# Sanasar1/Learning-Deep-Neural-Network-In-Distributed-Computing-Environment

Measured on AMD Instinct MI355X. Metric: samples/sec (whole node) + DP scaling eff., 3-layer MLP at 1/2/4/8 MI355X, higher is better.
Workload: dtype bf16

## Files before the change

learning-deep-neural-network-in-distributed-computing-environment_amd/csrc/bindings.cpp:

```cpp
#include <torch/extension.h>
#include <pybind11/stl.h>
#include <vector>
#include <cstring>
#include <string>
#include <mutex>
#include <map>
#include <ATen/hip/impl/HIPGuardImplMasqueradingAsCUDA.h>
#include <ATen/hip/impl/HIPStreamMasqueradingAsCUDA.h>

#include <rocprofiler-sdk-roctx/roctx.h>
#include "ldnn_kernels.h"

namespace {

hipStream_t cur_stream(const at::Tensor& t) {
  return c10::hip::getCurrentHIPStreamMasqueradingAsCUDA(t.device().index()).stream();
}

void check(hipError_t e, const char* what) {
  TORCH_CHECK(e == hipSuccess, "ldnn kernel '", what, "' failed: ", hipGetErrorString(e));
}

void check_dev(const at::Tensor& t, at::ScalarType dt, const char* name) {
  TORCH_CHECK(t.is_cuda(), name, " must be a GPU tensor");
// ... 950 lines not shown
  p.dlogits = bf16_mut(dlogits);
  p.stats = stats.data_ptr<float>();
  p.B = (int)B;
  p.C = (int)num_classes;
  p.ld = 16;
  p.grad_scale = (float)grad_scale;
  c10::hip::HIPGuardMasqueradingAsCUDA g(parts.device());
  check(ldnn::head_xent_parts(p, parts.data_ptr<float>(), (int)parts.size(0), cur_stream(parts)), "head_xent_parts");
}

void head_dgrad_stream(const at::Tensor& h, const at::Tensor& W, const at::Tensor& dlogits, const at::Tensor& dh,
                       const c10::optional<at::Tensor>& dbias, int64_t dgrad_epi) {
  check_dev(h, at::kBFloat16, "h");
  check_dev(W, at::kBFloat16, "W");
  check_dev(dlogits, at::kBFloat16, "dlogits");
  check_dev(dh, at::kBFloat16, "dh");
  const int64_t B = h.size(0), K = h.size(1);
  TORCH_CHECK(h.dim() == 2 && h.stride(1) == 1 && h.stride(0) % 8 == 0 && K % 8 == 0 && aligned16(h.data_ptr()),
              "head_dgrad_stream: h must be [B][K] with 16-B aligned rows");
  TORCH_CHECK(W.dim() == 2 && W.size(0) <= 16 && W.size(1) == K && W.stride(1) == 1 && W.stride(0) % 8 == 0 &&
                  aligned16(W.data_ptr()),
              "head_dgrad_stream: W must be [<= 16][K] with 16-B aligned rows");
  TORCH_CHECK(dlogits.is_contiguous() && dlogits.dim() == 2 && dlogits.size(0) == B && dlogits.size(1) == 16,
              "head_dgrad_stream: dlogits must be a contiguous [B][16] buffer");
  TORCH_CHECK(dh.dim() == 2 && dh.size(0) == B && dh.size(1) == K && dh.stride(1) == 1 && dh.stride(0) % 8 == 0 &&
                  aligned16(dh.data_ptr()),
              "head_dgrad_stream: dh must be [B][K] with 16-B aligned rows");
  TORCH_CHECK(dgrad_epi == ldnn::EPI_NONE || dgrad_epi == ldnn::EPI_DRELU || dgrad_epi == ldnn::EPI_DSIGMOID,
              "head_dgrad_stream: dgrad_epi must be EPI_NONE / EPI_DRELU / EPI_DSIGMOID");
  ldnn::HeadParams p{};
  p.h = bf16_ptr(h);
  p.W = bf16_ptr(W);
  p.dlogits = bf16_mut(dlogits);
  p.B = (int)B;
  p.K = (int)K;
  p.ld = 16;
  p.ldh = (int)h.stride(0);
  p.ldw = (int)W.stride(0);
  p.ldw_rows = (int)W.size(0);
  p.dh = bf16_mut(dh);
  p.lddh = (int)dh.stride(0);
  p.dgrad_epi = (int)dgrad_epi;
  if (dbias.has_value()) {
    check_dev(*dbias, at::kFloat, "dbias");
    TORCH_CHECK(dbias->is_contiguous() && dbias->numel() >= K, "head_dgrad_stream: bad dbias");
    p.dbias = dbias->data_ptr<float>();
  }
  c10::hip::HIPGuardMasqueradingAsCUDA g(h.device());
  check(ldnn::head_dgrad_stream(p, cur_stream(h)), "head_dgrad_stream");
}

void head_bwd(const at::Tensor& h, const at::Tensor& W, const at::Tensor& dlogits, const at::Tensor& dh,
              const at::Tensor& dW, const c10::optional<at::Tensor>& dbias, int64_t dgrad_epi,
              const c10::optional<at::Tensor>& db) {
  check_dev(h, at::kBFloat16, "h");
  check_dev(W, at::kBFloat16, "W");
  check_dev(dlogits, at::kBFloat16, "dlogits");
  check_dev(dh, at::kBFloat16, "dh");
  check_dev(dW, at::kFloat, "dW");
  const int64_t B = h.size(0), K = h.size(1);
  TORCH_CHECK(h.dim() == 2 && h.stride(1) == 1 && h.stride(0) % 8 == 0 && K % 64 == 0 && aligned16(h.data_ptr()),
              "head_bwd: h must be [B][K] with K % 64 == 0 and 16-B aligned rows");
  TORCH_CHECK(W.dim() == 2 && W.size(0) <= 16 && W.size(1) == K && W.stride(1) == 1, "head_bwd: W must be [<= 16][K]");
  TORCH_CHECK(dlogits.is_contiguous() && dlogits.dim() == 2 && dlogits.size(0) == B && dlogits.size(1) == 16 &&
                  aligned16(dlogits.data_ptr()),
              "head_bwd: dlogits must be a contiguous [B][16] buffer");
  TORCH_CHECK(dh.dim() == 2 && dh.size(0) == B && dh.size(1) == K && dh.stride(1) == 1 && dh.stride(0) % 8 == 0 &&
                  aligned16(dh.data_ptr()),
              "head_bwd: dh must be [B][K] with 16-B aligned rows");
  TORCH_CHECK(dgrad_epi == ldnn::EPI_NONE || dgrad_epi == ldnn::EPI_DRELU, "head_bwd: dgrad_epi must be EPI_NONE / EPI_DRELU");
  TORCH_CHECK(dW.dim() == 2 && dW.size(1) == K && dW.size(0) <= 16 && dW.stride(1) == 1, "head_bwd: dW must be [<= 16][K]");
  ldnn::HeadParams p{};
  p.h = bf16_ptr(h);
  p.W = bf16_ptr(W);
  p.dlogits = bf16_mut(dlogits);
  p.B = (int)B;
  p.K = (int)K;
  p.ld = 16;
  p.ldh = (int)h.stride(0);
  p.ldw = (int)W.stride(0);
  p.ldw_rows = (int)W.size(0);
  p.dh = bf16_mut(dh);
  p.lddh = (int)dh.stride(0);
  p.dgrad_epi = (int)dgrad_epi;
  p.dW = dW.data_ptr<float>();
  p.lddw = (int)dW.stride(0);
  p.nrows_w = (int)dW.size(0);
  if (dbias.has_value()) {
    check_dev(*dbias, at::kFloat, "dbias");
    TORCH_CHECK(dbias->is_contiguous() && dbias->numel() >= K, "head_bwd: bad dbias");
    p.dbias = dbias->data_ptr<float>();
  }
  if (db.has_value()) {
    check_dev(*db, at::kFloat, "db");
    TORCH_CHECK(db->is_contiguous() && db->numel() >= dW.size(0), "head_bwd: bad db");
    p.db = db->data_ptr<float>();
  }
  c10::hip::HIPGuardMasqueradingAsCUDA g(h.device());
  check(ldnn::head_bwd(p, cur_stream(h)), "head_bwd");
}

void head_wgrad(const at::Tensor& dz, const at::Tensor& h, const at::Tensor& dW, const c10::optional<at::Tensor>& db,
                int64_t splits) {
  check_dev(dz, at::kBFloat16, "dz");
  check_dev(h, at::kBFloat16, "h");
  check_dev(dW, at::kFloat, "dW");
  const int64_t B = h.size(0), K = h.size(1), ld = dz.size(1);
  TORCH_CHECK(dz.is_contiguous() && dz.size(0) == B && ld % 16 == 0 && ld <= 64, "head_wgrad: dz [B][ld], ld % 16 == 0");
  TORCH_CHECK(h.stride(1) == 1 && h.stride(0) % 8 == 0 && K % 8 == 0 && aligned16(h.data_ptr()), "head_wgrad: bad h");
  TORCH_CHECK(dW.dim() == 2 && dW.size(1) == K && dW.stride(1) == 1 && dW.size(0) <= ld && dW.stride(0) % 4 == 0 &&
                  aligned16(dW.data_ptr()),
              "head_wgrad: dW must be [rows <= ld][K] with 16-B aligned rows");
  ldnn::HeadWgradParams p{};
  p.dz = bf16_ptr(dz);
  p.h = bf16_ptr(h);
  p.dW = dW.data_ptr<float>();
  if (db.has_value()) {
    check_dev(*db, at::kFloat, "db");
    TORCH_CHECK(db->is_contiguous() && db->numel() >= dW.size(0), "head_wgrad: bad db");
    p.db = db->data_ptr<float>();
  }
  p.B = (int)B;
  p.K = (int)K;
  p.ld = (int)ld;
  p.ldh = (int)h.stride(0);
  p.lddw = (int)dW.stride(0);
  p.nrows = (int)dW.size(0);
  c10::hip::HIPGuardMasqueradingAsCUDA g(h.device());
  check(ldnn::head_wgrad(p, (int)splits, cur_stream(h)), "head_wgrad");
}

void bump_step(const at::Tensor& hp, const c10::optional<at::Tensor>& clip) {
  check_dev(hp, at::kFloat, "hp");
  TORCH_CHECK(hp.is_contiguous() && hp.numel() >= 2, "bump_step: hp must hold [lr, step]");
  check(ldnn::bump_step(hp.data_ptr<float>(), cur_stream(hp), clip_ptr(clip, hp)), "bump_step");
}

float* ema_hdr(const char* fn, const at::Tensor& hdr, const at::Tensor* like) {
  check_dev(hdr, at::kFloat, "hdr");
  TORCH_CHECK(hdr.is_contiguous() && hdr.numel() >= ldnn::kEmaState &&
                  (like == nullptr || hdr.device() == like->device()),
              fn, ": hdr must be a contiguous fp32 header of ", (int)ldnn::kEmaState,
              " elements on the buffers' device");
  return hdr.data_ptr<float>();
}

void ema_begin(const at::Tensor& hdr, const c10::optional<at::Tensor>& clip) {
  float* h = ema_hdr("ema_begin", hdr, nullptr);
  check(ldnn::ema_begin(h, cur_stream(hdr), clip_ptr(clip, hdr)), "ema_begin");
}

void lr_sched(const at::Tensor& hdr, const at::Tensor& hp, const c10::optional<at::Tensor>& clip) {
// ... 1207 lines not shown
        py::arg("chunks"), py::arg("partials"), py::arg("hp"), py::arg("grad_scale"), py::arg("beta1"),
        py::arg("beta2"), py::arg("eps"), py::arg("weight_decay"), py::arg("ranges"), py::arg("seg_offsets"),
        py::arg("clip") = py::none(), py::arg("policy") = (int64_t)1);
  m.def("lamb_finalize", &lamb_finalize, "per-segment LAMB trust ratios |w| / |u| and norms from lamb_moments' partials "
        "(+ ext sums); sums_out: the [2S] sums alone", py::arg("partials"), py::arg("segtab"), py::arg("ratio"),
        py::arg("w_norm"), py::arg("u_norm"), py::arg("ext") = py::none(), py::arg("clip") = py::none(),
        py::arg("sums_out") = py::none());
  m.def("lamb_apply", &lamb_apply, "LAMB apply pass: w -= lr * ratio * u over a 64-aligned range (+ bf16 shadow, "
        "gradient zero ranges)", py::arg("param"), py::arg("grad"), py::arg("m"), py::arg("v"), py::arg("shadow"),
        py::arg("hp"), py::arg("beta1"), py::arg("beta2"), py::arg("eps"), py::arg("weight_decay"), py::arg("ratio"),
        py::arg("map"), py::arg("zero_ranges") = std::vector<std::pair<int64_t, int64_t>>{},
        py::arg("clip") = py::none());
  m.def("adam_step", &adam_step, py::arg("param"), py::arg("grad"), py::arg("m"), py::arg("v"),
        py::arg("shadow"), py::arg("hp"), py::arg("grad_scale"), py::arg("beta1"), py::arg("beta2"),
        py::arg("eps"), py::arg("weight_decay"), py::arg("decoupled"),
        py::arg("zero_ranges") = std::vector<std::pair<int64_t, int64_t>>{}, py::arg("clip") = py::none());
  m.def("lion_step", &lion_step, "Lion: w = w (1 - lr wd) - lr sign(beta1 m + (1 - beta1) g), m = beta2 m + "
        "(1 - beta2) g (+ bf16 shadow, gradient zero ranges); lr = hp[0]", py::arg("param"), py::arg("grad"),
        py::arg("exp_avg"), py::arg("shadow"), py::arg("hp"), py::arg("grad_scale"), py::arg("beta1"),
        py::arg("beta2"), py::arg("weight_decay"),
        py::arg("zero_ranges") = std::vector<std::pair<int64_t, int64_t>>{}, py::arg("clip") = py::none());
  m.def("bump_step", &bump_step, py::arg("hp"), py::arg("clip") = py::none());
  m.def("lr_sched", &lr_sched, "learning-rate schedule, once per step: hp[0] = base * s(t + 1), the factor and the "
        "step count into hdr (nothing on a skipped step)", py::arg("hdr"), py::arg("hp"), py::arg("clip") = py::none());
  m.def("ema_begin", &ema_begin, "weight EMA, once per step: a_t and the update count into hdr (not on a skipped step)",
        py::arg("hdr"), py::arg("clip") = py::none());
  m.def("ema_update", &ema_update, "ema += a_t * (master - ema), a_t read from hdr", py::arg("master"),
        py::arg("ema"), py::arg("hdr"));
  m.def("ema_swap", &ema_swap, "master <-> ema (exact), shadow = bf16(new master)", py::arg("master"), py::arg("ema"),
        py::arg("shadow") = py::none());
  m.def("grad_sumsq", &grad_sumsq, "per-workgroup sums of squares of a flat fp32 range into partials[slot0 ...]; "
        "returns the number of slots written", py::arg("grad"), py::arg("partials"), py::arg("slot0") = 0);
  m.def("grad_sumsq_parts", &ldnn::grad_sumsq_parts, py::arg("n"));
  m.def("sumsq_total", &sumsq_total, py::arg("partials"), py::arg("nparts"), py::arg("out"));
  m.def("clip_finalize", &clip_finalize, "global-norm clipping state (coef / skip / norm / counters) from the "
        "partials (+ an external sum of squares)", py::arg("partials"), py::arg("nparts"), py::arg("state"),
        py::arg("grad_scale"), py::arg("ext") = py::none());
  m.def("set_opt_max_blocks", &ldnn::set_opt_max_blocks, py::arg("n"),
        "grid cap of optimizer launches from now on (0 = default)");
  m.def("head_fwd_xent", &head_fwd_xent, "fused narrow Linear + softmax-xent + argmax (per-16-row stats slots)",
        py::arg("h"), py::arg("W"), py::arg("bias"), py::arg("labels"), py::arg("logits"), py::arg("dlogits"),
        py::arg("stats"), py::arg("num_classes"), py::arg("grad_scale"), py::arg("dh") = py::none(), py::arg("dbias") = py::none(),
        py::arg("dgrad_epi") = (int64_t)ldnn::EPI_DRELU, py::arg("dbias_ws") = py::none(),
        py::arg("dgrad_mode") = (int64_t)-1);
  m.def("head_dgrad_ws_floats", &ldnn::head_dgrad_ws_floats, py::arg("B"), py::arg("K"));
  m.def("head_xent_parts", &head_xent_parts, "softmax-xent + argmax from EPI_BIAS_RELU_HEAD partial logits",
        py::arg("parts"), py::arg("bias"), py::arg("labels"), py::arg("logits"), py::arg("dlogits"), py::arg("stats"),
        py::arg("num_classes"), py::arg("grad_scale"));
  m.def("head_dgrad_stream", &head_dgrad_stream, "streaming head dgrad: dh = (dlogits W) * act'(h), dbias += colsums",
        py::arg("h"), py::arg("W"), py::arg("dlogits"), py::arg("dh"), py::arg("dbias") = py::none(),
        py::arg("dgrad_epi") = (int64_t)ldnn::EPI_DRELU);
  m.def("head_bwd", &head_bwd, "fused head dgrad + wgrad (dW / db / dbias accumulated: pre-cleared)", py::arg("h"),
        py::arg("W"), py::arg("dlogits"), py::arg("dh"), py::arg("dW"), py::arg("dbias") = py::none(),
        py::arg("dgrad_epi") = (int64_t)ldnn::EPI_DRELU, py::arg("db") = py::none());
  m.def("head_wgrad", &head_wgrad, "dW = dz^T h (+ db = colsum dz); splits > 1 accumulate atomically",
        py::arg("dz"), py::arg("h"), py::arg("dW"), py::arg("db") = py::none(), py::arg("splits") = 0);
  m.def("head_dgrad_max_k", &ldnn::head_dgrad_max_k);
  m.def("head_wgrad_splits", &ldnn::head_wgrad_splits, py::arg("B"), py::arg("K"));
  m.def("bn_fwd", &bn_fwd, py::arg("x"), py::arg("y"), py::arg("residual"), py::arg("gamma"), py::arg("beta"),
        py::arg("running_mean"), py::arg("running_var"), py::arg("save_mean"), py::arg("save_invstd"),
        py::arg("ws"), py::arg("eps"), py::arg("momentum"), py::arg("training"), py::arg("relu"),
        py::arg("num_batches") = py::none(), py::arg("stats_ready") = false, py::arg("mask") = py::none());
  m.def("bn_workspace_floats", &ldnn::bn_workspace_floats, "fp32 workspace of one BatchNorm (zero it once, keep it)",
        py::arg("C"));
  m.def("bn_bwd", &bn_bwd, py::arg("x"), py::arg("y"), py::arg("dy"), py::arg("dx"), py::arg("dres"),
        py::arg("gamma"), py::arg("save_mean"), py::arg("save_invstd"), py::arg("ws"), py::arg("dgamma"),
        py::arg("dbeta"), py::arg("relu"), py::arg("mask") = py::none(), py::arg("grad_assign") = false,
        py::arg("dy2") = py::none(), py::arg("stats_ready") = false);
  m.def("pool_fwd", &pool_fwd, py::arg("x"), py::arg("y"), py::arg("argmax"), py::arg("R"), py::arg("S"),
        py::arg("stride"), py::arg("pad"), py::arg("is_max"), py::arg("nchw_out") = false);
  m.def("pool_bwd", &pool_bwd, py::arg("dy"), py::arg("argmax"), py::arg("dx"), py::arg("R"), py::arg("S"),
        py::arg("stride"), py::arg("pad"), py::arg("is_max"), py::arg("dy2") = py::none(),
        py::arg("nchw_dy") = false);
  m.def("bn_dual_fwd", &bn_dual_fwd, "y = relu(bn_a(x) + bn_b(r)) in one pass (the shortcut BN output never stored)",
        py::arg("x"), py::arg("r"), py::arg("y"), py::arg("mask"), py::arg("gamma_a"), py::arg("beta_a"),
        py::arg("rm_a"), py::arg("rv_a"), py::arg("mean_a"), py::arg("invstd_a"), py::arg("ws_a"), py::arg("eps_a"),
        py::arg("mom_a"), py::arg("nb_a"), py::arg("ready_a"), py::arg("gamma_b"), py::arg("beta_b"),
        py::arg("rm_b"), py::arg("rv_b"), py::arg("mean_b"), py::arg("invstd_b"), py::arg("ws_b"), py::arg("eps_b"),
        py::arg("mom_b"), py::arg("nb_b"), py::arg("ready_b"));
  m.def("bn_dual_bwd", &bn_dual_bwd, "backward of bn_dual_fwd: dx, dr and both BNs' dgamma / dbeta",
        py::arg("x"), py::arg("r"), py::arg("y"), py::arg("mask"), py::arg("dy"), py::arg("dy2"), py::arg("dx"),
        py::arg("dr"), py::arg("gamma_a"), py::arg("mean_a"), py::arg("invstd_a"), py::arg("ws_a"),
        py::arg("dgamma_a"), py::arg("dbeta_a"), py::arg("assign_a"), py::arg("gamma_b"), py::arg("mean_b"),
        py::arg("invstd_b"), py::arg("ws_b"), py::arg("dgamma_b"), py::arg("dbeta_b"), py::arg("assign_b"));
  m.def("bn_pool_fwd", &bn_pool_fwd, "relu(BN(x)) -> 3x3/2 max-pool in one pass (pooled output + argmax)",
        py::arg("x"), py::arg("y"), py::arg("argmax"), py::arg("gamma"), py::arg("beta"), py::arg("running_mean"),
        py::arg("running_var"), py::arg("save_mean"), py::arg("save_invstd"), py::arg("ws"), py::arg("eps"),
        py::arg("momentum"), py::arg("num_batches") = py::none(), py::arg("stats_ready") = false,
        py::arg("pad") = 1, py::arg("xam") = py::none());
  m.def("bn_pool_bwd", &bn_pool_bwd, "backward of bn_pool_fwd: dx, dgamma / dbeta", py::arg("x"), py::arg("dy"),
        py::arg("argmax"), py::arg("dx"), py::arg("gamma"), py::arg("save_mean"), py::arg("save_invstd"),
        py::arg("ws"), py::arg("dgamma"), py::arg("dbeta"), py::arg("grad_assign") = false,
        py::arg("dy2") = py::none(), py::arg("pad") = 1, py::arg("xam") = py::none());
  m.def("gap_fwd", &gap_fwd);
  m.def("gap_bwd", &gap_bwd);
  m.def("set_conv_combine_last", &ldnn::set_conv_combine_last,
        "split-K combine summer: 1 = the tile's last K slice, 0 = the last workgroup to arrive", py::arg("on"));
  m.def("get_conv_combine_last", &ldnn::get_conv_combine_last);
  m.def("set_conv_bn_bwd", &ldnn::set_conv_bn_bwd,
        "dgrad-side BN backward statistics: 0 off, 1 slab sum only (default), 2 also the dgrad epilogue");
  m.def("get_conv_bn_bwd", &ldnn::get_conv_bn_bwd);
  m.def("gap_linear_ok", &ldnn::gap_linear_ok, "shapes the fused pooled classifier head takes", py::arg("N"),
        py::arg("HW"), py::arg("C"), py::arg("ncls"));
  m.def("gap_linear_fwd", &gap_linear_fwd, "global average pool + Linear (<= 16 classes) in one launch", py::arg("x"),
        py::arg("w"), py::arg("b"), py::arg("pooled"), py::arg("logits"), py::arg("ncls"));
  m.def("gap_linear_bwd", &gap_linear_bwd, "its backward: dW, db and the input gradient in one launch", py::arg("g"),
        py::arg("pooled"), py::arg("w"), py::arg("dw"), py::arg("db"), py::arg("dx"), py::arg("ncls"),
// ... 50 lines not shown
```

learning-deep-neural-network-in-distributed-computing-environment_amd/csrc/include/ldnn_kernels.h:

```cpp
#pragma once
#include <hip/hip_runtime.h>
#include <stdint.h>

namespace ldnn {

enum Epilogue : int {
  EPI_NONE = 0,
  EPI_BIAS = 1,
  EPI_BIAS_RELU = 2,
  EPI_BIAS_SIGMOID = 3,
  EPI_DRELU = 4,
  EPI_DSIGMOID = 5,
  EPI_OPT_SGD = 6,
  EPI_OPT_ADAM = 7,
  EPI_BIAS_RELU_MASK = 8,
  EPI_DRELU_MASK = 9,
  EPI_BIAS_RELU_HEAD = 10,
};

struct OptEpi {
  float* master;
  float* m;
  float* v;
  uint16_t* shadow;
// ... 302 lines not shown
int grad_sumsq_parts(int64_t n);
hipError_t grad_sumsq(const float* grad, int64_t n, float* partials, hipStream_t s);
hipError_t sumsq_total(const float* partials, int nparts, float* out, hipStream_t s);
hipError_t clip_finalize(const float* partials, int nparts, const float* ext, float* state, float grad_scale,
                         hipStream_t s);

int seg_sumsq_chunk();
hipError_t seg_sumsq(const float* master, const float* grad, int64_t n, const int32_t* chunks, int nchunks,
                     float* partials, hipStream_t s);
hipError_t trust_finalize(bool lamb, const float* partials, int nchunks, const int32_t* segtab, int S,
                          const float* ext, const float* hdr, const float* clip, float grad_scale, float weight_decay,
                          float* ratio, float* w_norm, float* g_norm, float* sums_out, hipStream_t s);

struct LambParams {
  float beta1, beta2, eps, weight_decay;
  GradZero zero;
};
hipError_t lamb_moments(const float* master, const float* grad, float* m, float* v, int64_t n, const int32_t* chunks,
                        int nchunks, const float* hp, float grad_scale, LambParams lp, float* partials,
                        hipStream_t s, const float* clip = nullptr, int policy = 1);
hipError_t lamb_apply(float* param, float* grad, const float* m, const float* v, uint16_t* shadow, const float* hp,
                      LambParams lp, int64_t n, const float* ratio, const uint16_t* map, hipStream_t s,
                      const float* clip = nullptr);

hipError_t lr_sched(float* hdr, float* hp, hipStream_t s, const float* clip = nullptr);

hipError_t ema_begin(float* hdr, hipStream_t s, const float* clip = nullptr);
hipError_t ema_update(const float* master, float* ema, const float* hdr, int64_t n, hipStream_t s);
hipError_t ema_swap(float* master, float* ema, uint16_t* shadow, int64_t n, hipStream_t s);

struct HeadParams {
  const uint16_t* h;
  const uint16_t* W;
  const float* bias;
  const int64_t* labels;
  uint16_t* logits;
  uint16_t* dlogits;
  float* stats;
  int B, K, C, ld, ldh, ldw, ldw_rows;
  float grad_scale;
  uint16_t* dh;
  float* dbias;
  float* dbias_ws;
  int lddh, dgrad_epi;
  int dgrad_mode;
  float* dW;
  float* db;
  int lddw, nrows_w;
};
hipError_t head_fwd_xent(const HeadParams& p, hipStream_t s);
hipError_t head_xent_parts(const HeadParams& p, const float* parts, int nparts, hipStream_t s);
hipError_t head_dgrad_stream(const HeadParams& p, hipStream_t s);
hipError_t head_bwd(const HeadParams& p, hipStream_t s);
int head_dgrad_max_k();
size_t head_dgrad_ws_floats(int B, int K);
hipError_t slab_sum(const float* ws, float* out, int64_t n4, int splits, float beta, hipStream_t s);
struct HeadWgradParams {
  const uint16_t* dz;
  const uint16_t* h;
  float* dW;
  float* db;
  int B, K, ld, ldh, lddw, nrows;
};
hipError_t head_wgrad(const HeadWgradParams& p, int splits, hipStream_t s);
int head_wgrad_splits(int B, int K);

hipError_t synth_normal_bf16(uint16_t* x, int64_t n, uint64_t seed, float stddev, hipStream_t s);
hipError_t synth_labels(int64_t* y, int64_t n, int classes, uint64_t seed, hipStream_t s);

constexpr int kAugOps = 15, kAugBins = 10, kAugPolicySlots = 64;
struct AugParams {
  const uint8_t* images;
  const int64_t* index;
  void* out;
  const float* a;
  const float* b;
  int64_t n_images;
  int B, C, H, W;
  uint64_t seed;
  int mode;
  int pad;
  int fixed_op, fixed_bin, fixed_sign;
  int n_policies;
  float mags[kAugOps][kAugBins];
  float rot_cos[kAugBins], rot_sin[kAugBins];
  int pol_op[kAugPolicySlots];
  float pol_prob[kAugPolicySlots];
  int pol_bin[kAugPolicySlots];
  int signed_op[kAugOps];
};
constexpr int kAugMaxPixels = 28 * 1024;
hipError_t augment_batch(const AugParams& p, bool out_f32, hipStream_t s);


constexpr int kIpcMaxRanks = 8;
constexpr int kIpcMaxBlocks = 256;
struct IpcPeers {
  const char* data[kIpcMaxRanks];
  uint32_t* sig[kIpcMaxRanks];
  char* mine;
  uint32_t* ctr;
  int* err;
  size_t half_bytes;
};
hipError_t oneshot_all_reduce(const IpcPeers& p, int rank, int world, int64_t n, bool bf16, void* buf, int blocks,
                              hipStream_t s);
// ... 3 lines not shown
```

learning-deep-neural-network-in-distributed-computing-environment_amd/csrc/kernels/head.hip:

```cpp
#include <algorithm>

#include <cstdlib>

#include "ldnn_common.h"
#include "ldnn_gemm_tile.h"
#include "ldnn_kernels.h"

namespace ldnn {

namespace {

constexpr int kFwdWaves = 8;

constexpr int kHeadDgradMaxK = 4096;

__device__ __forceinline__ int hs_off(int r, int q, int K) {
  return r * ((K + 127) & ~127) * 2 + ((q ^ (r & 15)) << 4);
}

template <int NT, bool DG>
__device__ __forceinline__ void head_softmax_xent(const HeadParams& p, floatx4 (&acc)[NT], floatx4 (*red)[NT][64],
                                                  int nred, float* dls, int lane, int row, int slot) {
#pragma unroll
  for (int j = 0; j < NT; ++j)
// ... 424 lines not shown
}

template <int DEPI>
hipError_t head_dgrad_dispatch(const HeadParams& p, hipStream_t s) {
  if (p.dgrad_mode == 0) {
    hipError_t e = launch_head_fwd<-1, false>(p, s);
    if (e != hipSuccess) return e;
    return launch_head_dgrad_stream<DEPI>(p, s);
  }
  hipError_t e = launch_head_fwd_dg<DEPI>(p, s);
  if (e != hipSuccess || p.dbias == nullptr) return e;
  return slab_sum(p.dbias_ws, p.dbias, p.K / 4, (p.B + 15) / 16, 1.f, s);
}

}

hipError_t head_fwd_xent(const HeadParams& p, hipStream_t s) {
  if (p.B <= 0) return hipSuccess;
  if (p.ld > 64 || p.ld % 16 != 0 || p.C > p.ld || p.ldw_rows > p.ld || p.K % 8 != 0) return hipErrorInvalidValue;
  if (p.dh == nullptr) return launch_head_fwd<-1, false>(p, s);
  if (p.lddh % 8 != 0) return hipErrorInvalidValue;
  if (p.dgrad_mode < 0 || p.dgrad_mode > 2 || (p.dgrad_mode == 0 && p.ld != 16)) return hipErrorInvalidValue;
  if ((p.dgrad_mode == 1 || p.dgrad_mode == 2) &&
      (p.K > kHeadDgradMaxK || (p.dbias != nullptr && p.dbias_ws == nullptr)))
    return hipErrorInvalidValue;
  switch (p.dgrad_epi) {
    case EPI_NONE: return head_dgrad_dispatch<EPI_NONE>(p, s);
    case EPI_DRELU: return head_dgrad_dispatch<EPI_DRELU>(p, s);
    case EPI_DSIGMOID: return head_dgrad_dispatch<EPI_DSIGMOID>(p, s);
    default: return hipErrorInvalidValue;
  }
}

hipError_t head_xent_parts(const HeadParams& p, const float* parts, int nparts, hipStream_t s) {
  if (p.B <= 0) return hipSuccess;
  if (p.ld != 16 || p.C > 16 || nparts < 1 || parts == nullptr) return hipErrorInvalidValue;
  const int slots = (p.B + 15) / 16;
  head_xent_parts_kernel<<<(slots + kPartWaves - 1) / kPartWaves, kPartWaves * 64, 0, s>>>(p, parts, nparts);
  return hipGetLastError();
}

hipError_t head_dgrad_stream(const HeadParams& p, hipStream_t s) {
  if (p.B <= 0) return hipSuccess;
  if (p.ld != 16 || p.dh == nullptr || p.lddh % 8 != 0 || p.K % 8 != 0 || p.ldw_rows > 16) return hipErrorInvalidValue;
  switch (p.dgrad_epi) {
    case EPI_NONE: return launch_head_dgrad_stream<EPI_NONE>(p, s);
    case EPI_DRELU: return launch_head_dgrad_stream<EPI_DRELU>(p, s);
    case EPI_DSIGMOID: return launch_head_dgrad_stream<EPI_DSIGMOID>(p, s);
    default: return hipErrorInvalidValue;
  }
}

typedef short s16x4 __attribute__((ext_vector_type(4)));
constexpr int kHbUnroll = 4;

template <bool RELU>
__global__ __launch_bounds__(256) void head_bwd_kernel(HeadParams p, int rows_per_wg) {
  constexpr int kH = 16 * 128, kD = 16 * 32, kSt = kH + kD;
  constexpr int kWave = kHbUnroll * kSt;
  __shared__ __attribute__((aligned(16))) char smem[4 * kWave];
  static_assert(4 * kWave >= 4 * 64 * 17 * 4, "the reduction scratch fits");
  const int lane = threadIdx.x & 63, wid = threadIdx.x >> 6;
  const int g = lane >> 4, r16 = lane & 15;
  const int n0 = blockIdx.x * 64;
  const int r_begin = blockIdx.y * rows_per_wg, r_end = min(p.B, r_begin + rows_per_wg);
  char* const st = smem + wid * kWave;
  typedef __attribute__((address_space(3))) bf16x4 lds_b4;

  s16x4 wa[4];
#pragma unroll
  for (int t = 0; t < 4; ++t) {
    const int n = n0 + (t >> 1) * 32 + 8 * (r16 >> 2) + (t & 1) * 4 + (r16 & 3);
#pragma unroll
    for (int q = 0; q < 4; ++q) {
      const int c = 4 * g + q;
      wa[t][q] = (c < p.ldw_rows && n < p.K) ? (short)p.W[(size_t)c * p.ldw + n] : (short)0;
    }
  }
  floatx4 acc2[4];
#pragma unroll
  for (int t = 0; t < 4; ++t) acc2[t] = floatx4{0.f, 0.f, 0.f, 0.f};
  float cs[16];
#pragma unroll
  for (int k = 0; k < 16; ++k) cs[k] = 0.f;
  float dbs[4] = {0.f, 0.f, 0.f, 0.f};
  const int q = r16 >> 2, pp = r16 & 3;

  for (int mb = r_begin + wid * 16; mb < r_end; mb += 64 * kHbUnroll) {
    u16x8 hv[kHbUnroll][2];
    uint2 dl[kHbUnroll];
#pragma unroll
    for (int u = 0; u < kHbUnroll; ++u) {
      const int m = mb + u * 64 + r16;
      hv[u][0] = hv[u][1] = u16x8{0, 0, 0, 0, 0, 0, 0, 0};
      dl[u] = uint2{0u, 0u};
      if (m < r_end) {
        const bf16_t* hr = p.h + (size_t)m * p.ldh + n0 + 8 * g;
        hv[u][0] = *reinterpret_cast<const u16x8*>(hr);
        hv[u][1] = *reinterpret_cast<const u16x8*>(hr + 32);
        dl[u] = *reinterpret_cast<const uint2*>(p.dlogits + (size_t)m * 16 + 4 * g);
      }
    }
#pragma unroll
    for (int u = 0; u < kHbUnroll; ++u) {
      char* sb = st + u * kSt;
      *reinterpret_cast<u16x8*>(sb + r16 * 128 + ((g ^ (r16 & 7)) << 4)) = hv[u][0];
      *reinterpret_cast<u16x8*>(sb + r16 * 128 + (((4 + g) ^ (r16 & 7)) << 4)) = hv[u][1];
      *reinterpret_cast<uint2*>(sb + kH + r16 * 32 + ((g ^ ((r16 >> 2) & 3)) << 3)) = dl[u];
    }
#pragma unroll
    for (int u = 0; u < kHbUnroll; ++u) {
      const int m = mb + u * 64 + r16;
      const s16x4 bl = __builtin_bit_cast(s16x4, dl[u]);
      floatx4 d[4];
#pragma unroll
      for (int t = 0; t < 4; ++t)
        d[t] = __builtin_amdgcn_mfma_f32_16x16x16bf16_1k(wa[t], bl, floatx4{0.f, 0.f, 0.f, 0.f}, 0, 0, 0);
      u16x8 o[2];
#pragma unroll
      for (int k = 0; k < 16; ++k) {
        const uint16_t hb = hv[u][k >> 3][k & 7];
        float v = d[k >> 2][k & 3];
        if constexpr (RELU) v = (short)hb > 0 ? v : 0.f;
        const uint16_t ob = f2bf(v);
        o[k >> 3][k & 7] = ob;
        cs[k] += bf2f(ob);
      }
      if (m < r_end) {
        bf16_t* dst = p.dh + (size_t)m * p.lddh + n0 + 8 * g;
        *reinterpret_cast<u16x8*>(dst) = o[0];
        *reinterpret_cast<u16x8*>(dst + 32) = o[1];
      }
#pragma unroll
      for (int c = 0; c < 4; ++c) dbs[c] += bf2f((uint16_t)((c < 2 ? dl[u].x : dl[u].y) >> (16 * (c & 1))));
    }
    __builtin_amdgcn_s_waitcnt(0xc07f);
    __builtin_amdgcn_wave_barrier();
#pragma unroll
    for (int u = 0; u < kHbUnroll; ++u) {
      const char* sb = st + u * kSt;
      const int row = 4 * g + q;
      const bf16x4 bd = __builtin_amdgcn_ds_read_tr16_b64_v4bf16((lds_b4*)(sb + kH + row * 32 + ((pp ^ g) << 3)));
#pragma unroll
      for (int nt = 0; nt < 4; ++nt) {
        const bf16x4 ah = __builtin_amdgcn_ds_read_tr16_b64_v4bf16(
            (lds_b4*)(sb + row * 128 + (((2 * nt + (pp >> 1)) ^ (row & 7)) << 4) + (pp & 1) * 8));
        acc2[nt] = __builtin_amdgcn_mfma_f32_16x16x16bf16_1k(__builtin_bit_cast(s16x4, ah),
                                                             __builtin_bit_cast(s16x4, bd), acc2[nt], 0, 0, 0);
      }
    }
  }

#pragma unroll
  for (int k = 0; k < 16; ++k)
#pragma unroll
    for (int o = 1; o < 16; o <<= 1) cs[k] += __shfl_xor(cs[k], o, 64);
#pragma unroll
  for (int q = 0; q < 4; ++q)
#pragma unroll
    for (int o = 1; o < 16; o <<= 1) dbs[q] += __shfl_xor(dbs[q], o, 64);
  __syncthreads();
  float* red = reinterpret_cast<float*>(smem);
#pragma unroll
  for (int nt = 0; nt < 4; ++nt)
#pragma unroll
    for (int r = 0; r < 4; ++r) red[(wid * 64 + lane) * 17 + nt * 4 + r] = acc2[nt][r];
  __syncthreads();
  if (wid == 0) {
#pragma unroll
    for (int nt = 0; nt < 4; ++nt)
#pragma unroll
      for (int r = 0; r < 4; ++r) {
        float t = 0.f;
#pragma unroll
        for (int w = 0; w < 4; ++w) t += red[(w * 64 + lane) * 17 + nt * 4 + r];
        const int n = n0 + 16 * nt + 4 * g + r;
        if (r16 < p.nrows_w && n < p.K) atomicAdd(p.dW + (size_t)r16 * p.lddw + n, t);
      }
  }
  __syncthreads();
  if (r16 == 0) {
#pragma unroll
    for (int k = 0; k < 16; ++k) red[(wid * 4 + g) * 17 + k] = cs[k];
    red[(wid * 4 + g) * 17 + 16] = 0.f;
#pragma unroll
    for (int q = 0; q < 4; ++q) red[16 * 17 + (wid * 4 + g) * 4 + q] = dbs[q];
  }
  __syncthreads();
  if (threadIdx.x < 64) {
    const int gg = threadIdx.x >> 4, k = threadIdx.x & 15;
    const int n = n0 + (k >> 3) * 32 + 8 * gg + (k & 7);
    if (p.dbias != nullptr && n < p.K) {
      float t = 0.f;
#pragma unroll
      for (int w = 0; w < 4; ++w) t += red[(w * 4 + gg) * 17 + k];
      atomicAdd(p.dbias + n, t);
    }
  } else if (threadIdx.x < 80 && blockIdx.x == 0 && p.db != nullptr) {
    const int c = threadIdx.x - 64, gg = c >> 2, q = c & 3;
    if (c < p.nrows_w) {
      float t = 0.f;
#pragma unroll
      for (int w = 0; w < 4; ++w) t += red[16 * 17 + (w * 4 + gg) * 4 + q];
      atomicAdd(p.db + c, t);
    }
  }
}

hipError_t head_bwd(const HeadParams& p, hipStream_t s) {
  if (p.B <= 0) return hipSuccess;
  if (p.ld != 16 || p.dh == nullptr || p.dW == nullptr || p.lddh % 8 != 0 || p.ldh % 8 != 0 || p.K % 64 != 0 ||
      p.ldw_rows > 16 || p.nrows_w > 16 || (p.dgrad_epi != EPI_NONE && p.dgrad_epi != EPI_DRELU))
    return hipErrorInvalidValue;
  const int gx = p.K / 64;
  constexpr int target = 768;
  int gy = std::max(1, std::min(256, target / gx));
  int rpw = (p.B + gy - 1) / gy;
  rpw = (rpw + 63) & ~63;
  gy = (p.B + rpw - 1) / rpw;
  const dim3 grid(gx, gy);
  if (p.dgrad_epi == EPI_DRELU) head_bwd_kernel<true><<<grid, 256, 0, s>>>(p, rpw);
  else head_bwd_kernel<false><<<grid, 256, 0, s>>>(p, rpw);
  return hipGetLastError();
}

size_t head_dgrad_ws_floats(int B, int K) { return (size_t)((B + 15) / 16) * K; }

int head_dgrad_max_k() { return kHeadDgradMaxK; }

int head_wgrad_splits(int B, int K) {
  const int cols = (K + kWgCols - 1) / kWgCols;
  int s = (256 + cols - 1) / cols;
  const int max_by_rows = B / (kWgWaves * kWgRows * 2);
  if (s > max_by_rows) s = max_by_rows;
  return s < 1 ? 1 : (s > 64 ? 64 : s);
}

hipError_t head_wgrad(const HeadWgradParams& p, int splits, hipStream_t s) {
  if (p.B <= 0 || p.K <= 0) return hipSuccess;
  if (p.ld > 64 || p.ld % 16 != 0 || p.nrows > p.ld || p.K % 8 != 0 || p.ldh % 8 != 0) return hipErrorInvalidValue;
  if (splits < 1) splits = head_wgrad_splits(p.B, p.K);
  const dim3 grid((p.K + kWgCols - 1) / kWgCols, splits), block(kWgWaves * 64);
  switch (p.ld / 16) {
    case 1: head_wgrad_kernel<1><<<grid, block, 0, s>>>(p); break;
    case 2: head_wgrad_kernel<2><<<grid, block, 0, s>>>(p); break;
    case 3: head_wgrad_kernel<3><<<grid, block, 0, s>>>(p); break;
    default: head_wgrad_kernel<4><<<grid, block, 0, s>>>(p); break;
  }
  return hipGetLastError();
}

}
```

Measured before the change: 10.31 million.

## Restructure head_bwd kernel to 128-column tiles with register-direct wgrad operands

```diff
diff --git a/learning-deep-neural-network-in-distributed-computing-environment_amd/csrc/bindings.cpp b/learning-deep-neural-network-in-distributed-computing-environment_amd/csrc/bindings.cpp
--- a/learning-deep-neural-network-in-distributed-computing-environment_amd/csrc/bindings.cpp
+++ b/learning-deep-neural-network-in-distributed-computing-environment_amd/csrc/bindings.cpp
@@ -1026,7 +1026,7 @@
 
 void head_bwd(const at::Tensor& h, const at::Tensor& W, const at::Tensor& dlogits, const at::Tensor& dh,
               const at::Tensor& dW, const c10::optional<at::Tensor>& dbias, int64_t dgrad_epi,
-              const c10::optional<at::Tensor>& db) {
+              const c10::optional<at::Tensor>& db, int64_t variant) {
   check_dev(h, at::kBFloat16, "h");
   check_dev(W, at::kBFloat16, "W");
   check_dev(dlogits, at::kBFloat16, "dlogits");
@@ -1071,7 +1071,7 @@
     p.db = db->data_ptr<float>();
   }
   c10::hip::HIPGuardMasqueradingAsCUDA g(h.device());
-  check(ldnn::head_bwd(p, cur_stream(h)), "head_bwd");
+  check(variant == 0 ? ldnn::head_bwd(p, cur_stream(h)) : ldnn::head_bwd_variant(p, (int)variant, cur_stream(h)), "head_bwd");
 }
 
 void head_wgrad(const at::Tensor& dz, const at::Tensor& h, const at::Tensor& dW, const c10::optional<at::Tensor>& db,
@@ -2385,7 +2385,7 @@
         py::arg("dgrad_epi") = (int64_t)ldnn::EPI_DRELU);
   m.def("head_bwd", &head_bwd, "fused head dgrad + wgrad (dW / db / dbias accumulated: pre-cleared)", py::arg("h"),
         py::arg("W"), py::arg("dlogits"), py::arg("dh"), py::arg("dW"), py::arg("dbias") = py::none(),
-        py::arg("dgrad_epi") = (int64_t)ldnn::EPI_DRELU, py::arg("db") = py::none());
+        py::arg("dgrad_epi") = (int64_t)ldnn::EPI_DRELU, py::arg("db") = py::none(), py::arg("variant") = 0);
   m.def("head_wgrad", &head_wgrad, "dW = dz^T h (+ db = colsum dz); splits > 1 accumulate atomically",
         py::arg("dz"), py::arg("h"), py::arg("dW"), py::arg("db") = py::none(), py::arg("splits") = 0);
   m.def("head_dgrad_max_k", &ldnn::head_dgrad_max_k);
diff --git a/learning-deep-neural-network-in-distributed-computing-environment_amd/csrc/include/ldnn_kernels.h b/learning-deep-neural-network-in-distributed-computing-environment_amd/csrc/include/ldnn_kernels.h
--- a/learning-deep-neural-network-in-distributed-computing-environment_amd/csrc/include/ldnn_kernels.h
+++ b/learning-deep-neural-network-in-distributed-computing-environment_amd/csrc/include/ldnn_kernels.h
@@ -378,6 +378,7 @@
 hipError_t head_xent_parts(const HeadParams& p, const float* parts, int nparts, hipStream_t s);
 hipError_t head_dgrad_stream(const HeadParams& p, hipStream_t s);
 hipError_t head_bwd(const HeadParams& p, hipStream_t s);
+hipError_t head_bwd_variant(const HeadParams& p, int variant, hipStream_t s);
 int head_dgrad_max_k();
 size_t head_dgrad_ws_floats(int B, int K);
 hipError_t slab_sum(const float* ws, float* out, int64_t n4, int splits, float beta, hipStream_t s);
diff --git a/learning-deep-neural-network-in-distributed-computing-environment_amd/csrc/kernels/head.hip b/learning-deep-neural-network-in-distributed-computing-environment_amd/csrc/kernels/head.hip
--- a/learning-deep-neural-network-in-distributed-computing-environment_amd/csrc/kernels/head.hip
+++ b/learning-deep-neural-network-in-distributed-computing-environment_amd/csrc/kernels/head.hip
@@ -500,176 +500,216 @@
 }
 
 typedef short s16x4 __attribute__((ext_vector_type(4)));
-constexpr int kHbUnroll = 4;
-
-template <bool RELU>
+typedef uint32_t u32x4 __attribute__((ext_vector_type(4)));
+
+constexpr int kHbUnroll = 2;
+constexpr int kHbRows = 4 * 16 * kHbUnroll;
+
+template <bool RELU, int XF>
 __global__ __launch_bounds__(256) void head_bwd_kernel(HeadParams p, int rows_per_wg) {
-  constexpr int kH = 16 * 128, kD = 16 * 32, kSt = kH + kD;
-  constexpr int kWave = kHbUnroll * kSt;
-  __shared__ __attribute__((aligned(16))) char smem[4 * kWave];
-  static_assert(4 * kWave >= 4 * 64 * 17 * 4, "the reduction scratch fits");
+  constexpr int U = kHbUnroll;
+  constexpr bool kStore = !(XF & 1), kMath = !(XF & 8), kWgrad = !(XF & (2 | 8)), kSums = !(XF & (4 | 8));
+  constexpr int kD = 16 * 32;
+  constexpr int kTr = 132;
+  constexpr int kWave = 16 * kTr * 4;
+  static_assert(U * kD <= kWave, "the dlogits staging fits the slice");
+  __shared__ __attribute__((aligned(16))) char smem[4 * kWave + 4 * (128 + 16) * 4];
   const int lane = threadIdx.x & 63, wid = threadIdx.x >> 6;
   const int g = lane >> 4, r16 = lane & 15;
-  const int n0 = blockIdx.x * 64;
+  const int n0 = blockIdx.x * 128;
+  const int nl = n0 + 8 * r16;
+  const bool cok = nl < p.K;
   const int r_begin = blockIdx.y * rows_per_wg, r_end = min(p.B, r_begin + rows_per_wg);
   char* const st = smem + wid * kWave;
   typedef __attribute__((address_space(3))) bf16x4 lds_b4;
 
-  s16x4 wa[4];
-#pragma unroll
-  for (int t = 0; t < 4; ++t) {
-    const int n = n0 + (t >> 1) * 32 + 8 * (r16 >> 2) + (t & 1) * 4 + (r16 & 3);
+  s16x4 wb[8];
+  {
+    const bool wvec = (reinterpret_cast<uintptr_t>(p.W) & 15) == 0 && p.ldw % 8 == 0;
+    u16x8 wr[4];
 #pragma unroll
     for (int q = 0; q < 4; ++q) {
       const int c = 4 * g + q;
-      wa[t][q] = (c < p.ldw_rows && n < p.K) ? (short)p.W[(size_t)c * p.ldw + n] : (short)0;
-    }
-  }
-  floatx4 acc2[4];
-#pragma unroll
-  for (int t = 0; t < 4; ++t) acc2[t] = floatx4{0.f, 0.f, 0.f, 0.f};
-  float cs[16];
-#pragma unroll
-  for (int k = 0; k < 16; ++k) cs[k] = 0.f;
+      wr[q] = u16x8{0, 0, 0, 0, 0, 0, 0, 0};
+      if (kMath && c < p.ldw_rows && cok) {
+        const bf16_t* wp = p.W + (size_t)c * p.ldw + nl;
+        if (wvec) {
+          wr[q] = *reinterpret_cast<const u16x8*>(wp);
+        } else {
+#pragma unroll
+          for (int t = 0; t < 8; ++t) wr[q][t] = wp[t];
+        }
+      }
+    }
+#pragma unroll
+    for (int t = 0; t < 8; ++t)
+#pragma unroll
+      for (int q = 0; q < 4; ++q) wb[t][q] = (short)wr[q][t];
+  }
+  floatx4 acc2[8];
+#pragma unroll
+  for (int t = 0; t < 8; ++t) acc2[t] = floatx4{0.f, 0.f, 0.f, 0.f};
+  float cs[8];
+#pragma unroll
+  for (int t = 0; t < 8; ++t) cs[t] = 0.f;
   float dbs[4] = {0.f, 0.f, 0.f, 0.f};
-  const int q = r16 >> 2, pp = r16 & 3;
-
-  for (int mb = r_begin + wid * 16; mb < r_end; mb += 64 * kHbUnroll) {
-    u16x8 hv[kHbUnroll][2];
-    uint2 dl[kHbUnroll];
-#pragma unroll
-    for (int u = 0; u < kHbUnroll; ++u) {
-      const int m = mb + u * 64 + r16;
-      hv[u][0] = hv[u][1] = u16x8{0, 0, 0, 0, 0, 0, 0, 0};
+  uint32_t chk = 0;
+  const int q4 = r16 >> 2, pp = r16 & 3;
+
+  for (int mb = r_begin + wid * 16 * U; mb < r_end; mb += kHbRows) {
+    u16x8 hv[U][4];
+    uint2 dl[U];
+#pragma unroll
+    for (int u = 0; u < U; ++u) {
+#pragma unroll
+      for (int r = 0; r < 4; ++r) {
+        const int m = mb + u * 16 + 4 * g + r;
+        hv[u][r] = u16x8{0, 0, 0, 0, 0, 0, 0, 0};
+        if (m < r_end && cok) hv[u][r] = *reinterpret_cast<const u16x8*>(p.h + (size_t)m * p.ldh + nl);
+      }
+      const int md = mb + u * 16 + r16;
       dl[u] = uint2{0u, 0u};
-      if (m < r_end) {
-        const bf16_t* hr = p.h + (size_t)m * p.ldh + n0 + 8 * g;
-        hv[u][0] = *reinterpret_cast<const u16x8*>(hr);
-        hv[u][1] = *reinterpret_cast<const u16x8*>(hr + 32);
-        dl[u] = *reinterpret_cast<const uint2*>(p.dlogits + (size_t)m * 16 + 4 * g);
-      }
-    }
-#pragma unroll
-    for (int u = 0; u < kHbUnroll; ++u) {
-      char* sb = st + u * kSt;
-      *reinterpret_cast<u16x8*>(sb + r16 * 128 + ((g ^ (r16 & 7)) << 4)) = hv[u][0];
-      *reinterpret_cast<u16x8*>(sb + r16 * 128 + (((4 + g) ^ (r16 & 7)) << 4)) = hv[u][1];
-      *reinterpret_cast<uint2*>(sb + kH + r16 * 32 + ((g ^ ((r16 >> 2) & 3)) << 3)) = dl[u];
-    }
-#pragma unroll
-    for (int u = 0; u < kHbUnroll; ++u) {
-      const int m = mb + u * 64 + r16;
-      const s16x4 bl = __builtin_bit_cast(s16x4, dl[u]);
-      floatx4 d[4];
-#pragma unroll
-      for (int t = 0; t < 4; ++t)
-        d[t] = __builtin_amdgcn_mfma_f32_16x16x16bf16_1k(wa[t], bl, floatx4{0.f, 0.f, 0.f, 0.f}, 0, 0, 0);
-      u16x8 o[2];
-#pragma unroll
-      for (int k = 0; k < 16; ++k) {
-        const uint16_t hb = hv[u][k >> 3][k & 7];
-        float v = d[k >> 2][k & 3];
-        if constexpr (RELU) v = (short)hb > 0 ? v : 0.f;
-        const uint16_t ob = f2bf(v);
-        o[k >> 3][k & 7] = ob;
-        cs[k] += bf2f(ob);
-      }
-      if (m < r_end) {
-        bf16_t* dst = p.dh + (size_t)m * p.lddh + n0 + 8 * g;
-        *reinterpret_cast<u16x8*>(dst) = o[0];
-        *reinterpret_cast<u16x8*>(dst + 32) = o[1];
-      }
-#pragma unroll
-      for (int c = 0; c < 4; ++c) dbs[c] += bf2f((uint16_t)((c < 2 ? dl[u].x : dl[u].y) >> (16 * (c & 1))));
-    }
-    __builtin_amdgcn_s_waitcnt(0xc07f);
-    __builtin_amdgcn_wave_barrier();
-#pragma unroll
-    for (int u = 0; u < kHbUnroll; ++u) {
-      const char* sb = st + u * kSt;
-      const int row = 4 * g + q;
-      const bf16x4 bd = __builtin_amdgcn_ds_read_tr16_b64_v4bf16((lds_b4*)(sb + kH + row * 32 + ((pp ^ g) << 3)));
-#pragma unroll
-      for (int nt = 0; nt < 4; ++nt) {
-        const bf16x4 ah = __builtin_amdgcn_ds_read_tr16_b64_v4bf16(
-            (lds_b4*)(sb + row * 128 + (((2 * nt + (pp >> 1)) ^ (row & 7)) << 4) + (pp & 1) * 8));
-        acc2[nt] = __builtin_amdgcn_mfma_f32_16x16x16bf16_1k(__builtin_bit_cast(s16x4, ah),
-                                                             __builtin_bit_cast(s16x4, bd), acc2[nt], 0, 0, 0);
-      }
-    }
-  }
-
-#pragma unroll
-  for (int k = 0; k < 16; ++k)
-#pragma unroll
-    for (int o = 1; o < 16; o <<= 1) cs[k] += __shfl_xor(cs[k], o, 64);
-#pragma unroll
-  for (int q = 0; q < 4; ++q)
-#pragma unroll
-    for (int o = 1; o < 16; o <<= 1) dbs[q] += __shfl_xor(dbs[q], o, 64);
+      if (md < r_end) dl[u] = *reinterpret_cast<const uint2*>(p.dlogits + (size_t)md * 16 + 4 * g);
+    }
+    if constexpr (kWgrad) {
+#pragma unroll
+      for (int u = 0; u < U; ++u)
+        *reinterpret_cast<uint2*>(st + u * kD + r16 * 32 + ((g ^ ((r16 >> 2) & 3)) << 3)) = dl[u];
+    }
+#pragma unroll
+    for (int u = 0; u < U; ++u) {
+      u16x8 o[4];
+      if constexpr (kMath) {
+        const s16x4 al = __builtin_bit_cast(s16x4, dl[u]);
+        floatx4 d[8];
+#pragma unroll
+        for (int t = 0; t < 8; ++t)
+          d[t] = __builtin_amdgcn_mfma_f32_16x16x16bf16_1k(al, wb[t], floatx4{0.f, 0.f, 0.f, 0.f}, 0, 0, 0);
+#pragma unroll
+        for (int r = 0; r < 4; ++r)
+#pragma unroll
+          for (int t = 0; t < 8; ++t) {
+            const uint16_t hb = hv[u][r][t];
+            float v = d[t][r];
+            if constexpr (RELU) v = (short)hb > 0 ? v : 0.f;
+            const uint16_t ob = f2bf(v);
+            o[r][t] = ob;
+            if constexpr (kSums) cs[t] += bf2f(ob);
+          }
+#pragma unroll
+        for (int c = 0; c < 4; ++c) dbs[c] += bf2f((uint16_t)((c < 2 ? dl[u].x : dl[u].y) >> (16 * (c & 1))));
+      } else {
+#pragma unroll
+        for (int r = 0; r < 4; ++r) o[r] = hv[u][r];
+      }
+#pragma unroll
+      for (int r = 0; r < 4; ++r) {
+        const int m = mb + u * 16 + 4 * g + r;
+        if constexpr (kStore) {
+          if (m < r_end && cok) *reinterpret_cast<u16x8*>(p.dh + (size_t)m * p.lddh + nl) = o[r];
+        } else {
+          const u32x4 c0 = __builtin_bit_cast(u32x4, o[r]);
+          chk ^= c0[0] ^ c0[1] ^ c0[2] ^ c0[3];
+        }
+      }
+    }
+    if constexpr (kWgrad) {
+      __builtin_amdgcn_s_waitcnt(0xc07f);
+      __builtin_amdgcn_wave_barrier();
+#pragma unroll
+      for (int u = 0; u < U; ++u) {
+        const int row = 4 * g + q4;
+        const bf16x4 bd = __builtin_amdgcn_ds_read_tr16_b64_v4bf16((lds_b4*)(st + u * kD + row * 32 + ((pp ^ g) << 3)));
+#pragma unroll
+        for (int t = 0; t < 8; ++t) {
+          const s16x4 ah = {(short)hv[u][0][t], (short)hv[u][1][t], (short)hv[u][2][t], (short)hv[u][3][t]};
+          acc2[t] = __builtin_amdgcn_mfma_f32_16x16x16bf16_1k(ah, __builtin_bit_cast(s16x4, bd), acc2[t], 0, 0, 0);
+        }
+      }
+    }
+  }
+  if (!kStore && chk == 0x9e3779b9u && r_begin < r_end && cok) p.dh[(size_t)r_begin * p.lddh + nl] = (bf16_t)chk;
+
+#pragma unroll
+  for (int t = 0; t < 8; ++t) {
+    cs[t] += __shfl_xor(cs[t], 16, 64);
+    cs[t] += __shfl_xor(cs[t], 32, 64);
+  }
+#pragma unroll
+  for (int c = 0; c < 4; ++c)
+#pragma unroll
+    for (int o = 1; o < 16; o <<= 1) dbs[c] += __shfl_xor(dbs[c], o, 64);
+  float* tr = reinterpret_cast<float*>(st);
+#pragma unroll
+  for (int t = 0; t < 8; ++t)
+#pragma unroll
+    for (int r = 0; r < 4; ++r) tr[r16 * kTr + 8 * (4 * g + r) + t] = acc2[t][r];
+  float* csum = reinterpret_cast<float*>(smem + 4 * kWave);
+  float* dsum = csum + 4 * 128;
+  if (g == 0) {
+#pragma unroll
+    for (int t = 0; t < 8; ++t) csum[wid * 128 + 8 * r16 + t] = cs[t];
+  }
+  if (r16 == 0) {
+#pragma unroll
+    for (int c = 0; c < 4; ++c) dsum[wid * 16 + 4 * g + c] = dbs[c];
+  }
   __syncthreads();
-  float* red = reinterpret_cast<float*>(smem);
-#pragma unroll
-  for (int nt = 0; nt < 4; ++nt)
-#pragma unroll
-    for (int r = 0; r < 4; ++r) red[(wid * 64 + lane) * 17 + nt * 4 + r] = acc2[nt][r];
-  __syncthreads();
-  if (wid == 0) {
-#pragma unroll
-    for (int nt = 0; nt < 4; ++nt)
-#pragma unroll
-      for (int r = 0; r < 4; ++r) {
-        float t = 0.f;
-#pragma unroll
-        for (int w = 0; w < 4; ++w) t += red[(w * 64 + lane) * 17 + nt * 4 + r];
-        const int n = n0 + 16 * nt + 4 * g + r;
-        if (r16 < p.nrows_w && n < p.K) atomicAdd(p.dW + (size_t)r16 * p.lddw + n, t);
-      }
-  }
-  __syncthreads();
-  if (r16 == 0) {
-#pragma unroll
-    for (int k = 0; k < 16; ++k) red[(wid * 4 + g) * 17 + k] = cs[k];
-    red[(wid * 4 + g) * 17 + 16] = 0.f;
-#pragma unroll
-    for (int q = 0; q < 4; ++q) red[16 * 17 + (wid * 4 + g) * 4 + q] = dbs[q];
-  }
-  __syncthreads();
-  if (threadIdx.x < 64) {
-    const int gg = threadIdx.x >> 4, k = threadIdx.x & 15;
-    const int n = n0 + (k >> 3) * 32 + 8 * gg + (k & 7);
-    if (p.dbias != nullptr && n < p.K) {
-      float t = 0.f;
-#pragma unroll
-      for (int w = 0; w < 4; ++w) t += red[(w * 4 + gg) * 17 + k];
-      atomicAdd(p.dbias + n, t);
-    }
-  } else if (threadIdx.x < 80 && blockIdx.x == 0 && p.db != nullptr) {
-    const int c = threadIdx.x - 64, gg = c >> 2, q = c & 3;
+  const float* tr0 = reinterpret_cast<const float*>(smem);
+#pragma unroll
+  for (int cc = 0; cc < 4; ++cc) {
+    const int c = 4 * wid + cc;
+    float t0 = 0.f, t1 = 0.f;
+#pragma unroll
+    for (int w = 0; w < 4; ++w) {
+      t0 += tr0[w * (kWave / 4) + c * kTr + lane];
+      t1 += tr0[w * (kWave / 4) + c * kTr + 64 + lane];
+    }
     if (c < p.nrows_w) {
-      float t = 0.f;
-#pragma unroll
-      for (int w = 0; w < 4; ++w) t += red[16 * 17 + (w * 4 + gg) * 4 + q];
-      atomicAdd(p.db + c, t);
-    }
-  }
-}
-
-hipError_t head_bwd(const HeadParams& p, hipStream_t s) {
+      atomicAdd(p.dW + (size_t)c * p.lddw + n0 + lane, t0);
+      if (n0 + 64 < p.K) atomicAdd(p.dW + (size_t)c * p.lddw + n0 + 64 + lane, t1);
+    }
+  }
+  if (threadIdx.x < 128) {
+    const int n = n0 + threadIdx.x;
+    if (p.dbias != nullptr && n < p.K)
+      atomicAdd(p.dbias + n, csum[threadIdx.x] + csum[128 + threadIdx.x] + csum[256 + threadIdx.x] + csum[384 + threadIdx.x]);
+  } else if (threadIdx.x < 144 && blockIdx.x == 0 && p.db != nullptr) {
+    const int c = threadIdx.x - 128;
+    if (c < p.nrows_w) atomicAdd(p.db + c, dsum[c] + dsum[16 + c] + dsum[32 + c] + dsum[48 + c]);
+  }
+}
+
+template <int XF>
+hipError_t launch_head_bwd(const HeadParams& p, hipStream_t s) {
   if (p.B <= 0) return hipSuccess;
   if (p.ld != 16 || p.dh == nullptr || p.dW == nullptr || p.lddh % 8 != 0 || p.ldh % 8 != 0 || p.K % 64 != 0 ||
       p.ldw_rows > 16 || p.nrows_w > 16 || (p.dgrad_epi != EPI_NONE && p.dgrad_epi != EPI_DRELU))
     return hipErrorInvalidValue;
-  const int gx = p.K / 64;
-  constexpr int target = 768;
-  int gy = std::max(1, std::min(256, target / gx));
+  const int gx = (p.K + 127) / 128;
+  constexpr int target = 512;
+  int gy = std::max(1, std::min(1024, target / gx));
   int rpw = (p.B + gy - 1) / gy;
-  rpw = (rpw + 63) & ~63;
+  rpw = (rpw + kHbRows - 1) / kHbRows * kHbRows;
   gy = (p.B + rpw - 1) / rpw;
   const dim3 grid(gx, gy);
-  if (p.dgrad_epi == EPI_DRELU) head_bwd_kernel<true><<<grid, 256, 0, s>>>(p, rpw);
-  else head_bwd_kernel<false><<<grid, 256, 0, s>>>(p, rpw);
+  if (p.dgrad_epi == EPI_DRELU) head_bwd_kernel<true, XF><<<grid, 256, 0, s>>>(p, rpw);
+  else head_bwd_kernel<false, XF><<<grid, 256, 0, s>>>(p, rpw);
   return hipGetLastError();
+}
+
+hipError_t head_bwd(const HeadParams& p, hipStream_t s) { return launch_head_bwd<0>(p, s); }
+
+hipError_t head_bwd_variant(const HeadParams& p, int variant, hipStream_t s) {
+  switch (variant) {
+    case 0: return launch_head_bwd<0>(p, s);
+    case 1: return launch_head_bwd<1>(p, s);
+    case 2: return launch_head_bwd<2>(p, s);
+    case 4: return launch_head_bwd<4>(p, s);
+    case 8: return launch_head_bwd<8>(p, s);
+    case 9: return launch_head_bwd<9>(p, s);
+    default: return hipErrorInvalidValue;
+  }
 }
 
 size_t head_dgrad_ws_floats(int B, int K) { return (size_t)((B + 15) / 16) * K; }
```

New measurement: 10.36 million, median of 6. About the same (+0.5%).
